# Ending2015a/dungeon_maps

Measured on NVIDIA B200. Metric: top-down maps/sec (batch 64, 640x480 depth + 16 semantic channels -> 400x400 maps), higher is better.
Workload: dtype f32

## Files before the change

dungeon_maps_b200/csrc/dm_labels.cu:

```cuda
#include <type_traits>

#include "dm_project.cuh"

namespace dm {

constexpr int kLblWarps = 8;
constexpr int kLblThreads = 32 * (kLblWarps + 1);
#ifndef DM_LBL_PROJ_J
#define DM_LBL_PROJ_J 1
#endif
constexpr int kLblProjJ = DM_LBL_PROJ_J;
constexpr int kLblTile = 128 * kLblWarps * kLblProjJ;
#ifndef DM_LBL_RES_K
#define DM_LBL_RES_K 2
#endif
constexpr int kLblResK = DM_LBL_RES_K;
constexpr int kLblResCells = 64 * kLblWarps * kLblResK;
#ifndef DM_LBL_RING
#define DM_LBL_RING 64
#endif
constexpr int kLblMaxRing = DM_LBL_RING;
constexpr int kLblList = 128 + 4;
constexpr uint32_t kKeyNegInf = 0x007fffffu;

struct LblPlan {
  int C, W2, CP, ring, lag, nsl;
  size_t slot_words, ctrl_bytes, flag_bytes;
  size_t workspace_bytes() const { return ctrl_bytes + flag_bytes + slot_words * 4 * (size_t)ring; }
};

static LblPlan make_lbl_plan(const DmProjCfg& cfg, int b) {
  LblPlan p{};
  p.C = cfg.C;
  p.W2 = (cfg.C + 1 <= 32) ? 1 : 2;
  p.CP = 1 + p.W2;
  const size_t M = (size_t)cfg.Mh * cfg.Mw;
  p.slot_words = (M * p.CP + 3) & ~(size_t)3;
  const int bb = b > 0 ? b : 1;
  p.ring = bb < kLblMaxRing ? bb : kLblMaxRing;
  if (p.ring < 2) p.ring = 2;
  p.lag = p.ring / 2;
  p.nsl = (int)((M + kSliceCells - 1) / kSliceCells);
  p.ctrl_bytes = ((size_t)(kCtrlWords + 2 * bb) * 4 + 255) & ~(size_t)255;
  p.flag_bytes = ((size_t)p.ring * p.nsl * kFlagStride * 4 + 255) & ~(size_t)255;
  return p;
}

struct LblDims {
  int C, CP, ring, lag, nsl, hasH;
  int vec_in;
  int vec_out;
  unsigned long long slot_words, ws_words;
};

struct LblItem {
  int kind, frame, idx, ok;
};

__device__ __forceinline__ uint32_t ld_stream_u32(const void* p) {
  uint32_t v;
  asm volatile("ld.global.nc.L1::no_allocate.u32 %0, [%1];" : "=r"(v) : "l"(p));
  return v;
}
__device__ __forceinline__ void red_or_u32(uint32_t* p, uint32_t v) {
  asm volatile("red.relaxed.gpu.global.or.b32 [%0], %1;" ::"l"(p), "r"(v) : "memory");
}

template <int W2>
using LblBits = std::conditional_t<W2 == 1, uint32_t, unsigned long long>;

struct LblQuad {
  float z[4];
  uint32_t lab, vm;
};

__device__ __forceinline__ LblQuad lbl_load_quad(const LblDims& d, const float* __restrict__ dframe,
                                                 const uint8_t* __restrict__ lframe, const uint8_t* __restrict__ vframe,
                                                 int n0, int N) {
  LblQuad q;
  q.z[0] = q.z[1] = q.z[2] = q.z[3] = 0.0f;
  q.lab = 0;
  q.vm = 0;
  if (n0 >= N) return q;
  if (d.vec_in && n0 + 3 < N) {
    const float4 z4 = ld_stream_f4(dframe + n0);
    q.z[0] = z4.x; q.z[1] = z4.y; q.z[2] = z4.z; q.z[3] = z4.w;
    q.lab = ld_stream_u32(lframe + n0);
    q.vm = vframe ? ld_stream_u32(vframe + n0) : 0x01010101u;
  } else {
#pragma unroll
    for (int k = 0; k < 4; ++k) {
      const bool in = n0 + k < N;
      q.z[k] = in ? ld_stream_f1(dframe + n0 + k) : 0.0f;
      q.lab |= (in ? (uint32_t)lframe[n0 + k] : 0u) << (8 * k);
      q.vm |= (in ? (vframe ? (uint32_t)(vframe[n0 + k] != 0) : 1u) : 0u) << (8 * k);
    }
  }
  return q;
}

template <int FAST, int W2>
__device__ __forceinline__ void lbl_proj_warp(const DmProjCfg& cfg, const LblDims& d, const DmProjSample& sp,
                                              const Rcps& rcp, const LblQuad& quad, int n0, int lane, uint32_t* list,
                                              uint32_t* __restrict__ acc, uint32_t slot_off,
                                              uint32_t* __restrict__ slot_flags) {
  using Bits = LblBits<W2>;
  const int N = cfg.H * cfg.W;
  int cl[4] = {-1, -1, -1, -1};
  float y[4] = {0.f, 0.f, 0.f, 0.f};
  Bits bt[4] = {0, 0, 0, 0};
  if (n0 < N) {
    const float* z = quad.z;
    const uint32_t lab = quad.lab, vm = quad.vm;
    const int r = n0 / cfg.W, c = n0 - r * cfg.W;
    if (FAST && c + 3 < cfg.W) {
      float xn[4];
#pragma unroll
      for (int k = 0; k < 4; ++k) xn[k] = div_by_rcp(__fsub_rn((float)(c + k), cfg.cx), cfg.fx, rcp.fx);
      const float yy = cfg.flip_h ? __fsub_rn((float)(cfg.H - 1), (float)r) : (float)r;
      const float yn = div_by_rcp(__fsub_rn(yy, cfg.cy), cfg.fy, rcp.fy);
      bool rowok = true;
      const int kb = cfg.clip_border;
      if (kb > 0) rowok = (r >= kb) && (r < cfg.H - kb);
#pragma unroll
      for (int k = 0; k < 4; ++k) {
        bool ok = rowok && (((vm >> (8 * k)) & 0xffu) != 0);
        if (kb > 0) ok = ok && (c + k >= kb) && (c + k < cfg.W - kb);
        cl[k] = pixel_cell_fast<FAST == 2, true>(cfg, sp, xn[k], yn, z[k], ok, &y[k], rcp.res);
      }
    } else {
      int rk = r, ck = c;
#pragma unroll
      for (int k = 0; k < 4; ++k) {
        cl[k] = pixel_cell(cfg, sp, rk, ck, z[k], ((vm >> (8 * k)) & 0xffu) != 0, &y[k]);
        if (++ck == cfg.W) { ck = 0; ++rk; }
      }
    }
#pragma unroll
    for (int k = 0; k < 4; ++k) {
      const int l = (int)((lab >> (8 * k)) & 0xffu);
      bt[k] = (Bits)1 << (l < cfg.C ? l : cfg.C);
    }
  }
  const bool p01 = (cl[0] >= 0) && (cl[0] == cl[1]);
  const bool p12 = (cl[1] >= 0) && (cl[1] == cl[2]);
  const bool p23 = (cl[2] >= 0) && (cl[2] == cl[3]);
  const bool t0 = (cl[0] >= 0) && !p01, t1 = (cl[1] >= 0) && !p12, t2 = (cl[2] >= 0) && !p23, t3 = cl[3] >= 0;
  y[1] = p01 ? fmaxf(y[0], y[1]) : y[1]; bt[1] = p01 ? (bt[0] | bt[1]) : bt[1];
  y[2] = p12 ? fmaxf(y[1], y[2]) : y[2]; bt[2] = p12 ? (bt[1] | bt[2]) : bt[2];
  y[3] = p23 ? fmaxf(y[2], y[3]) : y[3]; bt[3] = p23 ? (bt[2] | bt[3]) : bt[3];
// ... 460 lines not shown
```

dungeon_maps_b200/csrc/dm_project.cu:

```cuda
#include <cstdio>
#include <cstdlib>

#include <cuda.h>

#include "dm_project.cuh"

namespace dm {

constexpr int kProjThreads = 256;
constexpr int kResolveCells = 256;
#ifndef DM_MAX_RING
#define DM_MAX_RING 10
#endif
constexpr int kMaxRing = DM_MAX_RING;
constexpr size_t kRingBudgetBytes = (size_t)1 << 30;

struct ProjPlan {
  int Cv;
  int hasH;
  int CU;
  int CP;
  int rows;
  int tile;
  int ring;
  int lag;
  int nsl;
  size_t slot_words;
  size_t ctrl_bytes;
  size_t flag_bytes;
  size_t stage_bytes;
  size_t smem_tile;
  size_t smem_resolve;
  int ws_warps;
  int ws_groups;
  int ws_cg;
  int lean;
  int ws_r2d;
  size_t ws_stage_bytes;
  size_t smem_ws;
  size_t workspace_bytes() const { return ctrl_bytes + flag_bytes + slot_words * 4 * (size_t)ring; }
};

static int g_tile_rows = -1;
#ifndef DM_R2D_DEFAULT
#define DM_R2D_DEFAULT 0
#endif

static ProjPlan make_plan(const DmProjCfg& cfg, int b, int tile_rows = -1) {
  ProjPlan p{};
  p.Cv = cfg.C > 0 ? cfg.C : 1;
  p.hasH = (cfg.C > 0 && cfg.want_height) ? 1 : 0;
  p.CU = p.Cv + p.hasH;
  p.CP = (p.CU & 1) ? p.CU : p.CU + 1;
  p.rows = cfg.C + 1;
  const size_t M = (size_t)cfg.Mh * cfg.Mw;
  p.slot_words = (M * p.CP + 3) & ~(size_t)3;
  size_t ring = kRingBudgetBytes / (p.slot_words * 4);
  p.lean = cfg.C == 0 && g_tile_rows != -3;
  if (ring > (size_t)(p.lean ? 64 : kMaxRing)) ring = p.lean ? 64 : kMaxRing;
  if (ring > (size_t)(b > 0 ? b : 1)) ring = (size_t)(b > 0 ? b : 1);
  if (ring < 2) ring = 2;
  p.ring = (int)ring;
  p.lag = p.ring / 2;
  p.nsl = (int)((M + kSliceCells - 1) / kSliceCells);
  p.ctrl_bytes = ((size_t)(kCtrlWords + 2 * (b > 0 ? b : 1)) * 4 + 255) & ~(size_t)255;
  p.flag_bytes = ((size_t)p.ring * p.nsl * kFlagStride * 4 + 255) & ~(size_t)255;
  int tile = 1024;
  auto stage = [&](int t) { return (size_t)p.rows * (t + 4) * 4 + (size_t)t * 4; };
  while (tile > 128 && stage(tile) > (size_t)40 * 1024) tile >>= 1;
  p.tile = tile;
  p.stage_bytes = (stage(tile) + 127) & ~(size_t)127;
  p.smem_resolve = (size_t)kResolveCells * p.CP * 4;
  size_t st = p.stage_bytes > p.smem_resolve ? p.stage_bytes : ((p.smem_resolve + 127) & ~(size_t)127);
  p.stage_bytes = st;
  p.smem_tile = st + 256;
  auto ws_stage = [&](int ww, int rows) {
    size_t ws = ((size_t)rows * (128 * ww + 4) * 4 + (size_t)128 * ww * 4 + 127) & ~(size_t)127;
    const size_t ws_res = ((size_t)ww * 64 * p.CP * 4 + 127) & ~(size_t)127;
    return ws < ws_res ? ws_res : ws;
  };
  auto fits4 = [&](int ww, int rows) { return (ws_stage(ww, rows) + 256 + 1024) * 4 <= (size_t)228 * 1024; };
  p.ws_warps = 4;
  p.ws_groups = 1;
  if (!fits4(4, cfg.C + 1)) {
    p.ws_groups = (cfg.C + 23) / 24;
    p.ws_warps = 2;
  }
#ifdef DM_EXPERIMENT_KNOBS
  if (const char* e = getenv("DM_WS_WARPS")) {
    const int ww = atoi(e);
    if (ww == 2 || ww == 4) p.ws_warps = ww;
  }
  if (const char* e = getenv("DM_WS_GROUPS")) {
    const int g = atoi(e);
    if (g >= 1 && g <= 8) p.ws_groups = g;
  }
#endif
  if (cfg.C <= 0) p.ws_groups = 1;
  p.ws_cg = cfg.C > 0 ? (cfg.C + p.ws_groups - 1) / p.ws_groups : 0;
  p.ws_groups = cfg.C > 0 ? (cfg.C + p.ws_cg - 1) / p.ws_cg : 1;
  p.ws_r2d = tile_rows >= 0 ? tile_rows : g_tile_rows >= 0 ? g_tile_rows : DM_R2D_DEFAULT;
#ifdef DM_EXPERIMENT_KNOBS
  if (const char* e = getenv("DM_R2D")) if (tile_rows < 0) p.ws_r2d = atoi(e);
#endif
  if (p.ws_r2d != 0 && p.ws_r2d != 4 && p.ws_r2d != 8) p.ws_r2d = 0;
  if (p.ws_r2d == 8) {
    if (p.ws_groups == 1 && p.ws_warps == 4) p.ws_warps = 2; else p.ws_r2d = 4;
  }
  if (p.ws_r2d) {
    const size_t pw = (size_t)p.ws_r2d * 32 * p.ws_warps * 4;
    const size_t ws = (size_t)(p.ws_cg + 2) * pw;
    const size_t ws_res = ((size_t)p.ws_warps * 64 * p.CP * 4 + 127) & ~(size_t)127;
    p.ws_stage_bytes = ws < ws_res ? ws_res : ws;
    if (p.ws_cg > 256) p.ws_r2d = 0;
  }
  if (!p.ws_r2d) p.ws_stage_bytes = ws_stage(p.ws_warps, p.ws_cg + 1);
  p.smem_ws = p.ws_stage_bytes + 256;
  return p;
}

struct ProjDims {
  int Cv, hasH, CU, CP, rows, tile, ring, lag, nsl;
  unsigned long long slot_words;
  unsigned long long stage_bytes;
  int groups = 1, cg = 0;
  unsigned long long ws_words = 0;
};


__device__ __forceinline__ void phase_a(const uint8_t* __restrict__ vplane, const DmProjSample& sp,
                                        const DmProjCfg& cfg, int tile, int tile0, float* zrow, int* cells) {
  const int N = cfg.H * cfg.W;
  for (int q = threadIdx.x * 4; q < tile; q += kProjThreads * 4) {
    const int n0 = tile0 + q;
    int cl[4] = {-1, -1, -1, -1};
    float y[4] = {0.f, 0.f, 0.f, 0.f};
    if (n0 < N) {
      const float4 z4 = *reinterpret_cast<const float4*>(zrow + q);
      const float z[4] = {z4.x, z4.y, z4.z, z4.w};
      int r = n0 / cfg.W;
      int c = n0 - r * cfg.W;
#pragma unroll
      for (int k = 0; k < 4; ++k) {
        const bool ok = (n0 + k < N) && (vplane ? vplane[n0 + k] != 0 : true);
        cl[k] = pixel_cell(cfg, sp, r, c, z[k], ok, &y[k]);
        if (++c == cfg.W) { c = 0; ++r; }
      }
    }
    *reinterpret_cast<int4*>(cells + q) = make_int4(cl[0], cl[1], cl[2], cl[3]);
    *reinterpret_cast<float4*>(zrow + q) = make_float4(y[0], y[1], y[2], y[3]);
  }
}

template <bool IS_MIN>
__device__ __forceinline__ void emit_runs(const int* __restrict__ cells, const float* __restrict__ row,
                                          int beg, int end, float fill, uint32_t* __restrict__ acc_c, int CP) {
  int run_cell = -1;
  float run_v = fill;
  auto flush = [&]() {
    if (run_cell >= 0 && (IS_MIN ? (run_v < fill) : (run_v > fill)))
      atomicMax(acc_c + (size_t)run_cell * CP, IS_MIN ? ~enc(run_v) : enc(run_v));
  };
  auto visit = [&](int cl, float v) {
    if (cl >= 0) {
      if (cl != run_cell) {
        flush();
        run_cell = cl;
        run_v = fill;
      }
      run_v = IS_MIN ? fminf(run_v, v) : fmaxf(run_v, v);
    }
  };
  for (int i = beg; i < end; i += 4) {
    const int4 cl4 = *reinterpret_cast<const int4*>(cells + i);
    const float4 v4 = *reinterpret_cast<const float4*>(row + i);
    visit(cl4.x, v4.x);
    visit(cl4.y, v4.y);
    visit(cl4.z, v4.z);
    visit(cl4.w, v4.w);
  }
  flush();
}

// ... 139 lines not shown
  constexpr int RS = 128 * WW + 4;
  const int N = cfg.H * cfg.W;
  const int sb = cw * 128;
  const int q = sb + 4 * lane;
  const int n0 = it.tile0 + q;
  float* zrow = vals + nch * RS;
  int cl[4] = {-1, -1, -1, -1};
  float y[4] = {0.f, 0.f, 0.f, 0.f};
  if (n0 < N) {
    const float4 z4 = *reinterpret_cast<const float4*>(zrow + q);
    const float z[4] = {z4.x, z4.y, z4.z, z4.w};
    int c = it.c0 + q, r = it.r0;
    while (c >= cfg.W) { c -= cfg.W; ++r; }
    uint32_t vm = 0x01010101u;
    if (vplane) vm = *reinterpret_cast<const uint32_t*>(vplane + n0);
    if (FAST) {
      float xn[4];
#pragma unroll
      for (int k = 0; k < 4; ++k) xn[k] = div_by_rcp(__fsub_rn((float)(c + k), cfg.cx), cfg.fx, rcp.fx);
      const float yy = cfg.flip_h ? __fsub_rn((float)(cfg.H - 1), (float)r) : (float)r;
      const float yn = div_by_rcp(__fsub_rn(yy, cfg.cy), cfg.fy, rcp.fy);
      bool rowok = true;
      const int kb = cfg.clip_border;
      if (kb > 0) rowok = (r >= kb) && (r < cfg.H - kb);
#pragma unroll
      for (int k = 0; k < 4; ++k) {
        bool ok = rowok && (((vm >> (8 * k)) & 0xffu) != 0);
        if (kb > 0) ok = ok && (c + k >= kb) && (c + k < cfg.W - kb);
        cl[k] = pixel_cell_fast<FAST == 2, true>(cfg, sp, xn[k], yn, z[k], ok, &y[k], rcp.res);
      }
    } else {
#pragma unroll
      for (int k = 0; k < 4; ++k)
        cl[k] = pixel_cell(cfg, sp, r, c + k, z[k], ((vm >> (8 * k)) & 0xffu) != 0, &y[k]);
    }
  }
  const bool p01 = (cl[0] >= 0) && (cl[0] == cl[1]);
  const bool p12 = (cl[1] >= 0) && (cl[1] == cl[2]);
  const bool p23 = (cl[2] >= 0) && (cl[2] == cl[3]);
  const bool t0 = (cl[0] >= 0) && !p01, t1 = (cl[1] >= 0) && !p12, t2 = (cl[2] >= 0) && !p23, t3 = cl[3] >= 0;
  const int cnt = (int)t0 + (int)t1 + (int)t2 + (int)t3;
  int incl = cnt;
#pragma unroll
  for (int o = 1; o < 32; o <<= 1) {
    const int n = __shfl_up_sync(0xffffffffu, incl, o);
    if (lane >= o) incl += n;
  }
  const int total = __shfl_sync(0xffffffffu, incl, 31);
  const int padn = (4 - (total & 3)) & 3;
  const int o0 = sb + incl - cnt, o1 = o0 + (int)t0, o2 = o1 + (int)t1, o3 = o2 + (int)t2;
  if (t0) lcell[o0] = cl[0] * d.CP;
  if (t1) lcell[o1] = cl[1] * d.CP;
  if (t2) lcell[o2] = cl[2] * d.CP;
  if (t3) lcell[o3] = cl[3] * d.CP;
  {
    const int s0 = cl[0] >> 6, s1 = cl[1] >> 6, s2 = cl[2] >> 6, s3 = cl[3] >> 6;
    const int lastv = t3 ? s3 : t2 ? s2 : t1 ? s1 : t0 ? s0 : -1;
    int prev = __shfl_up_sync(0xffffffffu, lastv, 1);
    if (lane == 0) prev = -1;
    if (t0 && s0 != prev) st_flag(slot_flags + s0 * kFlagStride);
    prev = t0 ? s0 : prev;
    if (t1 && s1 != prev) st_flag(slot_flags + s1 * kFlagStride);
    prev = t1 ? s1 : prev;
    if (t2 && s2 != prev) st_flag(slot_flags + s2 * kFlagStride);
    prev = t2 ? s2 : prev;
    if (t3 && s3 != prev) st_flag(slot_flags + s3 * kFlagStride);
  }
  {
    const bool hmin = IS_MIN && cfg.C == 0;
    y[1] = p01 ? (hmin ? fminf(y[0], y[1]) : fmaxf(y[0], y[1])) : y[1];
    y[2] = p12 ? (hmin ? fminf(y[1], y[2]) : fmaxf(y[1], y[2])) : y[2];
    y[3] = p23 ? (hmin ? fminf(y[2], y[3]) : fmaxf(y[2], y[3])) : y[3];
    __syncwarp();
    if (t0) zrow[o0] = y[0];
    if (t1) zrow[o1] = y[1];
    if (t2) zrow[o2] = y[2];
    if (t3) zrow[o3] = y[3];
  }
  mbar_wait(full_vals, phase);
#ifdef DM_ABL_NOB
  return;
#endif
  [[maybe_unused]] const long long tp1 = DM_CLK();
#define DM_B1_ROW(ROW)                                                     \
  {                                                                        \
    float* row_ = (ROW);                                                   \
    float4 a = *reinterpret_cast<const float4*>(row_ + q);                 \
    a.y = p01 ? red2<IS_MIN>(a.x, a.y) : a.y;                              \
    a.z = p12 ? red2<IS_MIN>(a.y, a.z) : a.z;                              \
    a.w = p23 ? red2<IS_MIN>(a.z, a.w) : a.w;                              \
    __syncwarp();                                                          \
    if (t0) row_[o0] = a.x;                                                \
    if (t1) row_[o1] = a.y;                                                \
    if (t2) row_[o2] = a.z;                                                \
    if (t3) row_[o3] = a.w;                                                \
  }
  {
    int c = 0;
    for (; c + 4 <= nch; c += 4) {
      float* r0 = vals + c * RS;
      float4 a0 = *reinterpret_cast<const float4*>(r0 + q);
      float4 a1 = *reinterpret_cast<const float4*>(r0 + RS + q);
      float4 a2 = *reinterpret_cast<const float4*>(r0 + 2 * RS + q);
      float4 a3 = *reinterpret_cast<const float4*>(r0 + 3 * RS + q);
      a0.y = p01 ? red2<IS_MIN>(a0.x, a0.y) : a0.y; a1.y = p01 ? red2<IS_MIN>(a1.x, a1.y) : a1.y;
      a2.y = p01 ? red2<IS_MIN>(a2.x, a2.y) : a2.y; a3.y = p01 ? red2<IS_MIN>(a3.x, a3.y) : a3.y;
      a0.z = p12 ? red2<IS_MIN>(a0.y, a0.z) : a0.z; a1.z = p12 ? red2<IS_MIN>(a1.y, a1.z) : a1.z;
      a2.z = p12 ? red2<IS_MIN>(a2.y, a2.z) : a2.z; a3.z = p12 ? red2<IS_MIN>(a3.y, a3.z) : a3.z;
      a0.w = p23 ? red2<IS_MIN>(a0.z, a0.w) : a0.w; a1.w = p23 ? red2<IS_MIN>(a1.z, a1.w) : a1.w;
      a2.w = p23 ? red2<IS_MIN>(a2.z, a2.w) : a2.w; a3.w = p23 ? red2<IS_MIN>(a3.z, a3.w) : a3.w;
      __syncwarp();
      if (t0) { r0[o0] = a0.x; r0[RS + o0] = a1.x; r0[2 * RS + o0] = a2.x; r0[3 * RS + o0] = a3.x; }
      if (t1) { r0[o1] = a0.y; r0[RS + o1] = a1.y; r0[2 * RS + o1] = a2.y; r0[3 * RS + o1] = a3.y; }
      if (t2) { r0[o2] = a0.z; r0[RS + o2] = a1.z; r0[2 * RS + o2] = a2.z; r0[3 * RS + o2] = a3.z; }
      if (t3) { r0[o3] = a0.w; r0[RS + o3] = a1.w; r0[2 * RS + o3] = a2.w; r0[3 * RS + o3] = a3.w; }
    }
    for (; c < nch; ++c) DM_B1_ROW(vals + c * RS)
  }
#undef DM_B1_ROW
  __syncwarp();
  [[maybe_unused]] const long long tp2 = DM_CLK();
  const int total4 = total + padn;
  if (cfg.C > 0) {
    const int Cv = nch;
    const int cu_eff = Cv < 32 ? Cv : 32;
    const int streams = Cv <= 32 ? 32 / Cv : 1;
    const int passes = Cv <= 32 ? 1 : (Cv + 31) / 32;
    const int s = lane / cu_eff;
    const int per = ((total4 / 4 + streams - 1) / streams) * 4;
    const int beg = s * per;
    const int end = min(beg + per, total4);
    for (int pass = 0; pass < passes; ++pass) {
      const int c = pass * 32 + (lane - s * cu_eff);
      if (s >= streams || c >= Cv) continue;
      const float* row = vals + c * RS + sb;
      const int* lc = lcell + sb;
      const uint32_t off_c = slot_off + (uint32_t)(ch0 + c);
      const float fill = cfg.fill_value;
#ifdef DM_B2_BRANCHFREE
      if (beg >= end) continue;
      uint32_t pc = (uint32_t)lc[beg];
#else
      uint32_t pc = 0xffffffffu;
#endif
      float pv = fill;
      for (int i = beg; i < end; i += 4) {
        uint4 c4 = *reinterpret_cast<const uint4*>(lc + i);
        float4 v4 = *reinterpret_cast<const float4*>(row + i);
        if (i + 4 > total) {
          const int n = total - i;
          if (n < 2) { c4.y = c4.x; v4.y = fill; }
          if (n < 3) { c4.z = c4.y; v4.z = fill; }
          c4.w = c4.z; v4.w = fill;
        }
        const bool mp = pc == c4.x, m01 = c4.x == c4.y, m12 = c4.y == c4.z, m23 = c4.z == c4.w;
        red_key_if_run_ends<IS_MIN>(pc, c4.x, pv, fill, acc + (off_c + pc));
        v4.x = mp ? red2<IS_MIN>(pv, v4.x) : v4.x;
        v4.y = m01 ? red2<IS_MIN>(v4.x, v4.y) : v4.y;
        v4.z = m12 ? red2<IS_MIN>(v4.y, v4.z) : v4.z;
        v4.w = m23 ? red2<IS_MIN>(v4.z, v4.w) : v4.w;
        red_key_if_run_ends<IS_MIN>(c4.x, c4.y, v4.x, fill, acc + (off_c + c4.x));
        red_key_if_run_ends<IS_MIN>(c4.y, c4.z, v4.y, fill, acc + (off_c + c4.y));
        red_key_if_run_ends<IS_MIN>(c4.z, c4.w, v4.z, fill, acc + (off_c + c4.z));
        pc = c4.w;
        pv = v4.w;
      }
      red_key_if_run_ends<IS_MIN>(pc, 0xfffffffeu, pv, fill, acc + (off_c + pc));
    }
  }
  if ((d.hasH || cfg.C == 0) && ch0 == 0) {
    const bool hmin = IS_MIN && cfg.C == 0;
    const float hfill = cfg.C == 0 ? cfg.fill_value : -INFINITY;
    const uint32_t hoff = slot_off + (cfg.C == 0 ? 0u : (uint32_t)d.Cv);
    for (int base = 0; base < total; base += 32) {
      const int i = base + lane;
      const bool active = i < total;
      const uint32_t cellv = active ? (uint32_t)lcell[sb + i] : 0xffffffffu;
      float v = active ? zrow[sb + i] : hfill;
#pragma unroll
      for (int o = 1; o < 32; o <<= 1) {
        const float pv = __shfl_up_sync(0xffffffffu, v, o);
        const uint32_t pc = __shfl_up_sync(0xffffffffu, cellv, o);
        if (lane >= o && pc == cellv) v = hmin ? fminf(v, pv) : fmaxf(v, pv);
      }
      const uint32_t nc = __shfl_down_sync(0xffffffffu, cellv, 1);
      const bool last = lane == 31 || nc != cellv;
      const bool win = hmin ? (v < hfill) : (v > hfill);
      if (active && last && win) red_max_u32(acc + (hoff + cellv), hmin ? ~enc(v) : enc(v));
    }
  }
#ifdef DM_PROFILE
  [[maybe_unused]] const long long tp3 = DM_CLK();
  tprof[0] += tp1 - tp0; tprof[1] += tp2 - tp1; tprof[2] += tp3 - tp2; tprof[3] += total;
#endif
}

template <int FAST, bool IS_MIN, int WW, int R>
__device__ __forceinline__ void ws_proj_slice2d(const DmProjCfg& cfg, const ProjDims& d, const WsItem& it,
                                                const DmProjSample& sp, const Rcps& rcp,
                                                const uint8_t* __restrict__ vplane, float* vals, int* lcell,
                                                uint32_t* __restrict__ acc, uint32_t slot_off,
                                                uint32_t* __restrict__ slot_flags, int cw, int lane,
                                                uint64_t* full_vals, uint32_t phase, int ch0, int nch,
                                                long long* tprof) {
  [[maybe_unused]] const long long tp0 = DM_CLK();
  constexpr int TW = 32 * WW;
  constexpr int PW = R * TW;
  const int colt = (cw << 5) + lane;
  const int wbase = cw << 5;
  auto pos = [&](int i) { return (i >> 5) * TW + wbase + (i & 31); };
  float* zrow = vals + d.cg * PW;
  int cl[R];
  float y[R];
  {
    const int c = it.c0 + colt;
    const bool colok = c < cfg.W;
    float z[R];
#pragma unroll
    for (int k = 0; k < R; ++k) z[k] = zrow[k * TW + colt];
    const int kb = cfg.clip_border;
    bool ok[R];
#pragma unroll
    for (int k = 0; k < R; ++k) {
      const int r = it.r0 + k;
      ok[k] = colok && r < cfg.H;
      if (kb > 0) ok[k] = ok[k] && (r >= kb) && (r < cfg.H - kb) && (c >= kb) && (c < cfg.W - kb);
      if (vplane && ok[k]) ok[k] = vplane[(size_t)r * cfg.W + c] != 0;
    }
    if (FAST) {
      const float xn = div_by_rcp(__fsub_rn((float)c, cfg.cx), cfg.fx, rcp.fx);
#pragma unroll
      for (int k = 0; k < R; ++k) {
        const int r = it.r0 + k;
        const float yy = cfg.flip_h ? __fsub_rn((float)(cfg.H - 1), (float)r) : (float)r;
        const float yn = div_by_rcp(__fsub_rn(yy, cfg.cy), cfg.fy, rcp.fy);
        cl[k] = pixel_cell_fast<FAST == 2, true>(cfg, sp, xn, yn, z[k], ok[k], &y[k], rcp.res);
      }
    } else {
#pragma unroll
      for (int k = 0; k < R; ++k) {
        y[k] = 0.f;
        cl[k] = ok[k] ? pixel_cell(cfg, sp, it.r0 + k, c, z[k], true, &y[k]) : -1;
      }
    }
  }
  bool p[R], t[R];
#pragma unroll
  for (int k = 0; k < R; ++k) {
    p[k] = (k + 1 < R) && (cl[k] >= 0) && (cl[k] == cl[k + 1 < R ? k + 1 : k]);
    t[k] = (cl[k] >= 0) && !p[k];
  }
  int o[R];
  int total = 0;
  {
    const unsigned lt = (1u << lane) - 1u;
#pragma unroll
    for (int k = 0; k < R; ++k) {
      const unsigned bk = __ballot_sync(0xffffffffu, t[k]);
      o[k] = pos(total + __popc(bk & lt));
      total += __popc(bk);
    }
  }
  const int padn = (4 - (total & 3)) & 3;
#pragma unroll
  for (int k = 0; k < R; ++k)
    if (t[k]) lcell[o[k]] = cl[k] * d.CP;
  {
    int prev = -1;
#pragma unroll
    for (int k = 0; k < R; ++k) {
      const int sk = cl[k] >> 6;
      const int lk = __shfl_up_sync(0xffffffffu, t[k] ? sk : -1, 1);
      if (t[k] && sk != prev && (lane == 0 || sk != lk)) st_flag(slot_flags + sk * kFlagStride);
// ... 40 lines not shown
        for (int u = 0; u < CB; ++u)
          if (c + 4 * u < nch) {
#pragma unroll
            for (int k = 0; k < R; ++k)
              if (t[k]) pl[4 * u * PW + os[k]] = a[u][k];
          }
      }
    }
  }
  __syncwarp();
  [[maybe_unused]] const long long tp2 = DM_CLK();
  const int total4 = total + padn;
  if (cfg.C > 0) {
    const int Cv = nch;
    const int cu_eff = Cv < 32 ? Cv : 32;
    const int streams = Cv <= 32 ? 32 / Cv : 1;
    const int passes = Cv <= 32 ? 1 : (Cv + 31) / 32;
    const int s = lane / cu_eff;
    const int per = ((total4 / 4 + streams - 1) / streams) * 4;
    const int beg = s * per;
    const int end = min(beg + per, total4);
    for (int pass = 0; pass < passes; ++pass) {
      const int c = pass * 32 + (lane - s * cu_eff);
      if (s >= streams || c >= Cv) continue;
      const float* pl = vals + c * PW;
      const int swz = 4 * (c & 3);
      const uint32_t off_c = slot_off + (uint32_t)(ch0 + c);
      const float fill = cfg.fill_value;
      uint32_t pc = 0xffffffffu;
      float pv = fill;
      for (int i = beg; i < end; i += 4) {
        const int pi = pos(i);
        uint4 c4 = *reinterpret_cast<const uint4*>(lcell + pi);
        float4 v4 = *reinterpret_cast<const float4*>(pl + (pi ^ swz));
        if (i + 4 > total) {
          const int n = total - i;
          if (n < 2) { c4.y = c4.x; v4.y = fill; }
          if (n < 3) { c4.z = c4.y; v4.z = fill; }
          c4.w = c4.z; v4.w = fill;
        }
        const bool mp = pc == c4.x, m01 = c4.x == c4.y, m12 = c4.y == c4.z, m23 = c4.z == c4.w;
        red_key_if_run_ends<IS_MIN>(pc, c4.x, pv, fill, acc + (off_c + pc));
        v4.x = mp ? red2<IS_MIN>(pv, v4.x) : v4.x;
        v4.y = m01 ? red2<IS_MIN>(v4.x, v4.y) : v4.y;
        v4.z = m12 ? red2<IS_MIN>(v4.y, v4.z) : v4.z;
        v4.w = m23 ? red2<IS_MIN>(v4.z, v4.w) : v4.w;
        red_key_if_run_ends<IS_MIN>(c4.x, c4.y, v4.x, fill, acc + (off_c + c4.x));
        red_key_if_run_ends<IS_MIN>(c4.y, c4.z, v4.y, fill, acc + (off_c + c4.y));
        red_key_if_run_ends<IS_MIN>(c4.z, c4.w, v4.z, fill, acc + (off_c + c4.z));
        pc = c4.w;
        pv = v4.w;
      }
      red_key_if_run_ends<IS_MIN>(pc, 0xfffffffeu, pv, fill, acc + (off_c + pc));
    }
  }
  if ((d.hasH || cfg.C == 0) && ch0 == 0) {
    const bool hmin = IS_MIN && cfg.C == 0;
    const float hfill = cfg.C == 0 ? cfg.fill_value : -INFINITY;
    const uint32_t hoff = slot_off + (cfg.C == 0 ? 0u : (uint32_t)d.Cv);
    for (int base = 0; base < total; base += 32) {
      const int i = base + lane;
      const bool active = i < total;
      const int pi = pos(i);
      const uint32_t cellv = active ? (uint32_t)lcell[pi] : 0xffffffffu;
      float v = active ? zrow[pi] : hfill;
#pragma unroll
      for (int o2 = 1; o2 < 32; o2 <<= 1) {
        const float pv = __shfl_up_sync(0xffffffffu, v, o2);
        const uint32_t pc = __shfl_up_sync(0xffffffffu, cellv, o2);
        if (lane >= o2 && pc == cellv) v = hmin ? fminf(v, pv) : fmaxf(v, pv);
      }
      const uint32_t nc = __shfl_down_sync(0xffffffffu, cellv, 1);
      const bool last = lane == 31 || nc != cellv;
      const bool win = hmin ? (v < hfill) : (v > hfill);
      if (active && last && win) red_max_u32(acc + (hoff + cellv), hmin ? ~enc(v) : enc(v));
    }
  }
#ifdef DM_PROFILE
  [[maybe_unused]] const long long tp3 = DM_CLK();
  tprof[0] += tp1 - tp0; tprof[1] += tp2 - tp1; tprof[2] += tp3 - tp2; tprof[3] += total;
#endif
}

__device__ __forceinline__ bool ws_resolve_slice(uint32_t* __restrict__ acc_slot, const DmProjCfg& cfg,
                                                 const ProjDims& d, uint32_t* __restrict__ slot_flags, int frame,
                                                 int cell_tile, int tile_cells, int cw, int lane, uint32_t* wres,
                                                 float* __restrict__ topdown,
                                                 uint8_t* __restrict__ mask, float* __restrict__ height) {
  const int M = cfg.Mh * cfg.Mw;
  const int cell0 = cell_tile * tile_cells + cw * 64;
  const int ncell = min(64, M - cell0);
  if (ncell <= 0) return false;
  uint32_t* slice_flag = slot_flags + (size_t)(cell0 >> 6) * kFlagStride;
  const int nw = ncell * d.CP;
  const int nw4 = nw & ~3;
  uint32_t* src = acc_slot + (size_t)cell0 * d.CP;
  uint32_t any = 0;
  uint32_t flagged = 0;
  if (lane == 0) {
    flagged = __ldcg(slice_flag);
    if (flagged) __stcg(slice_flag, 0u);
  }
  flagged = __shfl_sync(0xffffffffu, flagged, 0);
  if (!flagged) {
    if (!(ncell == 64 && (M & 3) == 0))
      for (int k = lane; k < nw; k += 32) wres[k] = 0;
  } else {
  for (int base = 0; base < nw4; base += 512) {
    uint4 v[4];
#pragma unroll
    for (int u = 0; u < 4; ++u) {
      const int i = base + (u * 32 + lane) * 4;
      v[u] = i < nw4 ? __ldcg(reinterpret_cast<const uint4*>(src + i)) : make_uint4(0, 0, 0, 0);
    }
#pragma unroll
    for (int u = 0; u < 4; ++u) {
      const int i = base + (u * 32 + lane) * 4;
      const uint32_t nz = v[u].x | v[u].y | v[u].z | v[u].w;
      any |= nz;
      if (i < nw4) {
        if (nz) __stcg(reinterpret_cast<uint4*>(src + i), make_uint4(0, 0, 0, 0));
        *reinterpret_cast<uint4*>(wres + i) = v[u];
      }
    }
  }
  for (int k = nw4 + lane; k < nw; k += 32) {
    const uint32_t v = __ldcg(src + k);
    if (v) __stcg(src + k, 0u);
    wres[k] = v;
    any |= v;
  }
  }
  const bool occupied = __any_sync(0xffffffffu, any != 0);
  const size_t plane0 = (size_t)frame * d.Cv * M + cell0;
  if (!occupied && ncell == 64 && (M & 3) == 0) {
    const float f = cfg.fill_value;
    const float4 f4 = make_float4(f, f, f, f);
    for (int c = lane >> 4; c < d.Cv; c += 2) st_stream_f4(topdown + plane0 + (size_t)c * M + (lane & 15) * 4, f4);
    if ((M & 15) == 0) {
      for (int c = lane >> 2; c < d.Cv; c += 8) st_stream_u4(mask + plane0 + (size_t)c * M + (lane & 3) * 16, 0u);
    } else {
      for (int c = lane >> 4; c < d.Cv; c += 2) st_stream_u32(mask + plane0 + (size_t)c * M + (lane & 15) * 4, 0u);
    }
    if (d.hasH && lane < 16)
      st_stream_f4(height + (size_t)frame * M + cell0 + lane * 4, make_float4(-INFINITY, -INFINITY, -INFINITY, -INFINITY));
    return flagged != 0;
  }
  __syncwarp();
  for (int j = lane; j < ncell; j += 32) {
    const uint32_t* mine = wres + j * d.CP;
    float* tp = topdown + plane0 + j;
    uint8_t* mp = mask + plane0 + j;
    for (int c = 0; c < d.Cv; ++c) {
      const uint32_t k = mine[c];
      const float out = k ? dec_red(k, cfg.reduction) : cfg.fill_value;
      st_stream_f1(tp, out);
      st_stream_u8(mp, k ? 1 : 0);
      tp += M;
      mp += M;
    }
    if (d.hasH) {
      const uint32_t k = mine[d.Cv];
      st_stream_f1(height + (size_t)frame * M + cell0 + j, k ? dec(k) : -INFINITY);
    }
  }
  __syncwarp();
  return flagged != 0;
}

template <int FAST, bool IS_MIN, int WW, int R2D>
#ifndef DM_WS_MINB
#define DM_WS_MINB 0
#endif
__global__ void __launch_bounds__(32 * (WW + 1), (R2D == 4 && WW == 4) ? 6 : DM_WS_MINB)
proj_ws_kernel(const float* __restrict__ depth, const float* __restrict__ values,
               const uint8_t* __restrict__ valid, const DmProjSample* __restrict__ samples,
               const DmProjCfg cfg, const ProjDims d, int b, uint32_t* __restrict__ ctrl,
               uint32_t* __restrict__ flags, uint32_t* __restrict__ acc, float* __restrict__ topdown,
               uint8_t* __restrict__ mask, float* __restrict__ height, const ProjGuard guard,
               const __grid_constant__ CUtensorMap tmv, const __grid_constant__ CUtensorMap tmd) {
  extern __shared__ __align__(128) unsigned char smem[];
  constexpr int kWsWarps = WW, kWsTile = 128 * WW, kWsResolveCells = 64 * WW * kResK;
  constexpr int RS = kWsTile + 4;
  constexpr int TW = 32 * WW;
  constexpr int PW = (R2D ? R2D : 1) * TW;
  const Rcps rcp{__frcp_rn(cfg.map_res), __frcp_rn(cfg.fx), __frcp_rn(cfg.fy)};
  unsigned char* stage = smem;
  unsigned char* tail = smem + d.stage_bytes;
  uint64_t* full = reinterpret_cast<uint64_t*>(tail);
  uint64_t* empty = full + 1;
  uint64_t* full_vals = reinterpret_cast<uint64_t*>(tail + 24);
  WsItem* item = reinterpret_cast<WsItem*>(tail + 32);
  DmProjSample* sps = reinterpret_cast<DmProjSample*>(tail + 64);

  const int tid = threadIdx.x, lane = tid & 31, warp = tid >> 5;
  const int N = cfg.H * cfg.W, M = cfg.Mh * cfg.Mw;
  const int CBk = (cfg.W + TW - 1) / TW;
  const int P = (R2D ? ((cfg.H + R2D - 1) / (R2D ? R2D : 1)) * CBk : (N + kWsTile - 1) / kWsTile) * d.groups;
  const int R = (M + kWsResolveCells - 1) / kWsResolveCells;
  uint32_t* proj_done = ctrl + kCtrlWords;
  uint32_t* resolve_done = proj_done + b;
  uint32_t* occ_count = reinterpret_cast<uint32_t*>(tail + 16);

  int lag = d.lag;
  {
    const uint32_t hint = __ldcg(ctrl + 4);
    if (hint) {
      const float touched = (float)(hint - 1u) * (1.0f / 65536.0f) * (float)d.slot_words * 4.0f;
      const int fit = (int)fminf((float)(48u << 20) / fmaxf(touched, 1.0f), 64.0f) - 2;
      lag = max(min(2, d.lag), min(fit, d.lag));
    }
  }
  const int ahead = lag >= 3 ? 2 : 1;
  const int ring = min(d.ring, 2 * lag);
  const unsigned total = (unsigned)(b + lag) * (unsigned)(P + R);

  if (tid == 0) {
    *occ_count = 0;
    mbar_init(full, 1);
    mbar_init(full_vals, 1);
    mbar_init(empty, kWsWarps);
    asm volatile("fence.mbarrier_init.release.cluster;" ::: "memory");
  }
  __syncthreads();

  if (warp == kWsWarps) {
    const uint64_t policy = policy_evict_first();
    int pend_kind = kItemNone, pend_frame = 0;
    uint32_t fills = 0;
    [[maybe_unused]] long long pp[4] = {0, 0, 0, 0};
    unsigned raw0 = 0, raw1 = 0;
    if (lane == 0) {
      raw0 = atomicAdd(ctrl, 1u);
      if (ahead == 2) raw1 = atomicAdd(ctrl, 1u);
    }
    while (true) {
      [[maybe_unused]] const long long tq0 = DM_CLK();
      const unsigned t = __shfl_sync(0xffffffffu, raw0, 0);
      if (lane == 0) {
        if (ahead == 2) {
          raw0 = raw1;
          if (t < total) raw1 = atomicAdd(ctrl, 1u);
        } else if (t < total) {
          raw0 = atomicAdd(ctrl, 1u);
        }
      }
      WsItem it{};
      it.ok = 1;
      if (t >= total) {
        it.kind = kItemExit;
      } else {
        decode_ticket(t, b, P, R, lag, &it.kind, &it.frame, &it.idx);
      }
      const uint32_t* dep = nullptr;
      uint32_t dep_target = 0;
      uint32_t spw0 = 0, spw1 = 0;
      if (it.kind == kItemProj) {
// ... 476 lines not shown
```

dungeon_maps_b200/csrc/dm_project.cuh:

```cuda
#pragma once

#include "dm_common.cuh"

namespace dm {

constexpr int kSliceCells = 64;
#ifndef DM_FLAG_STRIDE
#define DM_FLAG_STRIDE 8
#endif
constexpr int kFlagStride = DM_FLAG_STRIDE;
constexpr int kCtrlWords = 512;
constexpr unsigned long long kSpinLimitNs = 4000000000ull;
#ifndef DM_SUSPEND_NS
#define DM_SUSPEND_NS 20000u
#endif

struct ProjGuard {
  unsigned long long spin_ns;
  uint32_t dep_bias;
  uint32_t* status;
};
ProjGuard proj_guard(int device);
bool take_timeout(int device);

// ... 47 lines not shown
__device__ __forceinline__ uint64_t policy_evict_first() {
  uint64_t p;
  asm volatile("createpolicy.fractional.L2::evict_first.b64 %0, 1.0;" : "=l"(p));
  return p;
}
__device__ __forceinline__ uint32_t ld_acquire(const uint32_t* p) {
  uint32_t v;
  asm volatile("ld.acquire.gpu.global.u32 %0, [%1];" : "=r"(v) : "l"(p) : "memory");
  return v;
}
__device__ __forceinline__ uint32_t ld_relaxed(const uint32_t* p) {
  uint32_t v;
  asm volatile("ld.relaxed.gpu.global.u32 %0, [%1];" : "=r"(v) : "l"(p) : "memory");
  return v;
}
__device__ __forceinline__ unsigned long long globaltimer() {
  unsigned long long t;
  asm volatile("mov.u64 %0, %globaltimer;" : "=l"(t));
  return t;
}
__device__ __forceinline__ bool wait_count(const uint32_t* counter, uint32_t target, uint32_t* ctrl,
                                           unsigned long long spin_ns) {
  if (ld_acquire(counter) >= target) return true;
  const unsigned long long t0 = globaltimer();
  while (ld_acquire(counter) < target) {
    __nanosleep(64);
    if (globaltimer() - t0 > spin_ns) {
      atomicExch(ctrl + 2, 1u);
      return false;
    }
  }
  return true;
}

__device__ __forceinline__ void red_release_add1(uint32_t* p) {
  asm volatile("red.release.gpu.global.add.u32 [%0], 1;" ::"l"(p) : "memory");
}

__device__ __forceinline__ void scrub_after_timeout(uint32_t* ctrl, uint32_t* flags, unsigned long long words, int tid,
                                                    int nthreads, uint32_t* status) {
  if (__ldcg(ctrl + 2) == 0u) return;
  uint4* w4 = reinterpret_cast<uint4*>(flags);
  for (unsigned long long i = tid; i < words / 4; i += nthreads) __stcg(w4 + i, make_uint4(0u, 0u, 0u, 0u));
  __threadfence();
  if (tid == 0 && status) {
    asm volatile("st.relaxed.sys.global.u32 [%0], %1;" ::"l"(status), "r"(1u) : "memory");
    __threadfence_system();
  }
}

enum { kItemProj = 0, kItemResolve = 1, kItemNone = 2, kItemExit = 3 };

__device__ __forceinline__ void decode_ticket(unsigned t, int b, int P, int R, int lag, int* kind, int* frame,
                                              int* idx) {
  const unsigned per = (unsigned)(P + R);
  const int s = (int)(t / per);
  const int j = (int)(t - (unsigned)s * per);
  const unsigned rb0 = (unsigned)(((unsigned long long)j * (unsigned)R) / per);
  const unsigned rb1 = (unsigned)(((unsigned long long)(j + 1) * (unsigned)R) / per);
  if (rb1 > rb0) {
    *kind = kItemResolve;
    *idx = (int)rb0;
  } else {
    *kind = kItemProj;
    *idx = j - (int)rb0;
  }
  *frame = *kind == kItemProj ? s : s - lag;
  if (*frame < 0 || *frame >= b) *kind = kItemNone;
}

__device__ __forceinline__ void mbar_arrive(uint64_t* bar) {
  asm volatile("mbarrier.arrive.shared::cta.b64 _, [%0];" ::"r"(smem_u32(bar)) : "memory");
}

__device__ __forceinline__ void st_flag(uint32_t* p) {
  asm volatile("st.relaxed.gpu.global.u32 [%0], %1;" ::"l"(p), "r"(1u) : "memory");
}
__device__ __forceinline__ void red_max_u32(uint32_t* p, uint32_t v) {
#ifdef DM_ABL_NORED
  asm volatile("" ::"l"(p), "r"(v) : "memory");
#else
  asm volatile("red.relaxed.gpu.global.max.u32 [%0], %1;" ::"l"(p), "r"(v) : "memory");
#endif
}
template <bool IS_MIN>
__device__ __forceinline__ void red_key_if_run_ends(uint32_t ca, uint32_t cb, float v, float fill, uint32_t* p) {
  const uint32_t key = IS_MIN ? ~enc(v) : enc(v);
#ifdef DM_ABL_NORED
  asm volatile("" ::"r"(ca), "r"(cb), "f"(v), "f"(fill), "l"(p), "r"(key) : "memory");
#elif defined(DM_B2_BRANCHFREE)
  {
    const bool on = (ca != cb) && (IS_MIN ? (v < fill) : (v > fill));
    asm volatile("red.relaxed.gpu.global.max.u32 [%0], %1;" ::"l"(p), "r"(on ? key : 0u) : "memory");
  }
#elif defined(DM_ABL_REDVAR)
  {
    const int ln = threadIdx.x & 31;
    bool on = (ca != cb) && (IS_MIN ? (v < fill) : (v > fill));
#if DM_ABL_REDVAR == 2
    on = on && ((ln & 1) == 0);
#elif DM_ABL_REDVAR == 4
    on = on && ((ln & 15) == 0);
#endif
#if DM_ABL_REDVAR == 3
    p = reinterpret_cast<uint32_t*>((reinterpret_cast<unsigned long long>(p) & ~0xfffffffull) | (reinterpret_cast<unsigned long long>(p) & 0xffffcull));
#endif
#if DM_ABL_REDVAR == 1
    if (on) asm volatile("st.relaxed.gpu.global.u32 [%0], %1;" ::"l"(p), "r"(key) : "memory");
#else
    if (on) asm volatile("red.relaxed.gpu.global.max.u32 [%0], %1;" ::"l"(p), "r"(key) : "memory");
#endif
  }
#else
  if (IS_MIN)
    asm volatile(
        "{\n\t.reg .pred p;\n\t"
        "setp.ne.u32 p, %0, %1;\n\t"
        "setp.lt.and.f32 p, %2, %3, p;\n\t"
        "@p red.relaxed.gpu.global.max.u32 [%4], %5;\n\t}" ::"r"(ca), "r"(cb), "f"(v), "f"(fill), "l"(p), "r"(key) : "memory");
  else
    asm volatile(
        "{\n\t.reg .pred p;\n\t"
        "setp.ne.u32 p, %0, %1;\n\t"
        "setp.gt.and.f32 p, %2, %3, p;\n\t"
        "@p red.relaxed.gpu.global.max.u32 [%4], %5;\n\t}" ::"r"(ca), "r"(cb), "f"(v), "f"(fill), "l"(p), "r"(key) : "memory");
#endif
}
__device__ __forceinline__ void red_max_u32_if(bool pred, uint32_t* p, uint32_t v) {
  asm volatile(
      "{\n\t.reg .pred p;\n\t"
      "setp.ne.b32 p, %0, 0;\n\t"
      "@p red.global.max.u32 [%1], %2;\n\t}" ::"r"((int)pred), "l"(p), "r"(v) : "memory");
}

__device__ __forceinline__ float div_by_rcp(float x, float res, float rres) {
  const float q0 = __fmul_rn(x, rres);
  const float q1 = __fmaf_rn(__fmaf_rn(-q0, res, x), rres, q0);
  return __fmaf_rn(__fmaf_rn(-q1, res, x), rres, q1);
}

template <bool GLOBAL, bool RCP_DIV = false>
__device__ __forceinline__ int pixel_cell_fast(const DmProjCfg& cfg, const DmProjSample& sp, float xn, float yn,
                                               float z, bool ok, float* y_out, float rres = 0.0f) {
  if (cfg.has_trunc_depth_max) ok = ok && (z <= cfg.trunc_depth_max);
  if (cfg.has_trunc_depth_min) ok = ok && (z >= cfg.trunc_depth_min);
  const float X = __fmul_rn(xn, z), Y = __fmul_rn(yn, z);
  const float* Rl = sp.to_local.R;
  float ly = __fmaf_rn(Rl[7], z, __fmul_rn(Rl[4], Y));
  float lz = __fmaf_rn(Rl[8], z, __fmul_rn(Rl[5], Y));
  ly = __fadd_rn(ly, sp.to_local.t[1]);
  if (cfg.has_trunc_height_max) ok = ok && (ly <= cfg.trunc_height_max);
  float gx = X, gz = lz;
  if (GLOBAL) {
    const float* Rg = sp.to_global.R;
    gx = __fadd_rn(__fmaf_rn(Rg[6], lz, __fmul_rn(Rg[0], X)), sp.to_global.t[0]);
    gz = __fadd_rn(__fmaf_rn(Rg[8], lz, __fmul_rn(Rg[2], X)), sp.to_global.t[2]);
  }
  float xf, zf;
  if (RCP_DIV) {
    const float res = cfg.map_res;
    const float xb = __fadd_rn(div_by_rcp(gx, res, rres), sp.width_offset);
    float zb = __fadd_rn(div_by_rcp(gz, res, rres), sp.height_offset);
    if (cfg.flip_h) zb = __fsub_rn((float)(cfg.Mh - 1), zb);
    xf = floorf(__fadd_rn(xb, 0.5f));
    zf = floorf(__fadd_rn(zb, 0.5f));
  } else {
// ... 20 lines not shown
```

Measured before the change: 137,100.

## Add binary-value presence bitmask path for semantic channel projection

Checks at runtime whether every semantic value in a warp's tile is exactly 0 or 1. When so, it packs per-pixel channel bits into one presence word per cell group and issues a single red.or per cell run instead of per-channel red.max operations. The resolve stage then expands the presence bits back into per-channel keys. This widens the cell slot by the number of groups, rescales the ring cap to keep memory similar, changes lag rounding, and sets a min-blocks launch bound for the R2D=0 path. The aim is to cut global atomic traffic for one-hot or binary labels, at the cost of extra detection work and a larger slot.

After: 139,200 (median of 6 runs). 1.02x the previous value.

```diff
diff --git a/dungeon_maps_b200/csrc/dm_labels.cu b/dungeon_maps_b200/csrc/dm_labels.cu
--- a/dungeon_maps_b200/csrc/dm_labels.cu
+++ b/dungeon_maps_b200/csrc/dm_labels.cu
@@ -62,10 +62,6 @@
   asm volatile("ld.global.nc.L1::no_allocate.u32 %0, [%1];" : "=r"(v) : "l"(p));
   return v;
 }
-__device__ __forceinline__ void red_or_u32(uint32_t* p, uint32_t v) {
-  asm volatile("red.relaxed.gpu.global.or.b32 [%0], %1;" ::"l"(p), "r"(v) : "memory");
-}
-
 template <int W2>
 using LblBits = std::conditional_t<W2 == 1, uint32_t, unsigned long long>;
 
diff --git a/dungeon_maps_b200/csrc/dm_project.cu b/dungeon_maps_b200/csrc/dm_project.cu
--- a/dungeon_maps_b200/csrc/dm_project.cu
+++ b/dungeon_maps_b200/csrc/dm_project.cu
@@ -1,5 +1,6 @@
 #include <cstdio>
 #include <cstdlib>
+#include <type_traits>
 
 #include <cuda.h>
 
@@ -51,17 +52,48 @@
   p.Cv = cfg.C > 0 ? cfg.C : 1;
   p.hasH = (cfg.C > 0 && cfg.want_height) ? 1 : 0;
   p.CU = p.Cv + p.hasH;
-  p.CP = (p.CU & 1) ? p.CU : p.CU + 1;
   p.rows = cfg.C + 1;
   const size_t M = (size_t)cfg.Mh * cfg.Mw;
+  auto ws_rows = [&](int ww, int rows) {
+    return ((size_t)rows * (128 * ww + 4) * 4 + (size_t)128 * ww * 4 + 127) & ~(size_t)127;
+  };
+  auto ws_stage = [&](int ww, int rows) {
+    const size_t ws = ws_rows(ww, rows);
+    const size_t ws_res = ((size_t)ww * 64 * p.CP * 4 + 127) & ~(size_t)127;
+    return ws < ws_res ? ws_res : ws;
+  };
+  auto fits4 = [&](int ww, int rows) { return (ws_rows(ww, rows) + 256 + 1024) * 4 <= (size_t)228 * 1024; };
+  p.ws_warps = 4;
+  p.ws_groups = 1;
+  if (!fits4(4, cfg.C + 1)) {
+    p.ws_groups = (cfg.C + 23) / 24;
+    p.ws_warps = 2;
+  }
+#ifdef DM_EXPERIMENT_KNOBS
+  if (const char* e = getenv("DM_WS_WARPS")) {
+    const int ww = atoi(e);
+    if (ww == 2 || ww == 4) p.ws_warps = ww;
+  }
+  if (const char* e = getenv("DM_WS_GROUPS")) {
+    const int g = atoi(e);
+    if (g >= 1 && g <= 8) p.ws_groups = g;
+  }
+#endif
+  if (cfg.C <= 0) p.ws_groups = 1;
+  p.ws_cg = cfg.C > 0 ? (cfg.C + p.ws_groups - 1) / p.ws_groups : 0;
+  p.ws_groups = cfg.C > 0 ? (cfg.C + p.ws_cg - 1) / p.ws_cg : 1;
+  const int cp_keys = (p.CU & 1) ? p.CU : p.CU + 1;
+  const int cell_words = p.CU + (cfg.C > 0 ? p.ws_groups : 0);
+  p.CP = (cell_words & 1) ? cell_words : cell_words + 1;
   p.slot_words = (M * p.CP + 3) & ~(size_t)3;
   size_t ring = kRingBudgetBytes / (p.slot_words * 4);
   p.lean = cfg.C == 0 && g_tile_rows != -3;
-  if (ring > (size_t)(p.lean ? 64 : kMaxRing)) ring = p.lean ? 64 : kMaxRing;
+  const size_t cap = p.lean ? 64 : ((size_t)kMaxRing * cp_keys + p.CP / 2) / p.CP;
+  if (ring > cap) ring = cap;
   if (ring > (size_t)(b > 0 ? b : 1)) ring = (size_t)(b > 0 ? b : 1);
   if (ring < 2) ring = 2;
   p.ring = (int)ring;
-  p.lag = p.ring / 2;
+  p.lag = (p.ring + 1) / 2;
   p.nsl = (int)((M + kSliceCells - 1) / kSliceCells);
   p.ctrl_bytes = ((size_t)(kCtrlWords + 2 * (b > 0 ? b : 1)) * 4 + 255) & ~(size_t)255;
   p.flag_bytes = ((size_t)p.ring * p.nsl * kFlagStride * 4 + 255) & ~(size_t)255;
@@ -74,31 +106,6 @@
   size_t st = p.stage_bytes > p.smem_resolve ? p.stage_bytes : ((p.smem_resolve + 127) & ~(size_t)127);
   p.stage_bytes = st;
   p.smem_tile = st + 256;
-  auto ws_stage = [&](int ww, int rows) {
-    size_t ws = ((size_t)rows * (128 * ww + 4) * 4 + (size_t)128 * ww * 4 + 127) & ~(size_t)127;
-    const size_t ws_res = ((size_t)ww * 64 * p.CP * 4 + 127) & ~(size_t)127;
-    return ws < ws_res ? ws_res : ws;
-  };
-  auto fits4 = [&](int ww, int rows) { return (ws_stage(ww, rows) + 256 + 1024) * 4 <= (size_t)228 * 1024; };
-  p.ws_warps = 4;
-  p.ws_groups = 1;
-  if (!fits4(4, cfg.C + 1)) {
-    p.ws_groups = (cfg.C + 23) / 24;
-    p.ws_warps = 2;
-  }
-#ifdef DM_EXPERIMENT_KNOBS
-  if (const char* e = getenv("DM_WS_WARPS")) {
-    const int ww = atoi(e);
-    if (ww == 2 || ww == 4) p.ws_warps = ww;
-  }
-  if (const char* e = getenv("DM_WS_GROUPS")) {
-    const int g = atoi(e);
-    if (g >= 1 && g <= 8) p.ws_groups = g;
-  }
-#endif
-  if (cfg.C <= 0) p.ws_groups = 1;
-  p.ws_cg = cfg.C > 0 ? (cfg.C + p.ws_groups - 1) / p.ws_groups : 0;
-  p.ws_groups = cfg.C > 0 ? (cfg.C + p.ws_cg - 1) / p.ws_cg : 1;
   p.ws_r2d = tile_rows >= 0 ? tile_rows : g_tile_rows >= 0 ? g_tile_rows : DM_R2D_DEFAULT;
 #ifdef DM_EXPERIMENT_KNOBS
   if (const char* e = getenv("DM_R2D")) if (tile_rows < 0) p.ws_r2d = atoi(e);
@@ -404,6 +411,7 @@
   return;
 #endif
   [[maybe_unused]] const long long tp1 = DM_CLK();
+  uint32_t nbo = 0, nbt = 0;
 #define DM_B1_ROW(ROW)                                                     \
   {                                                                        \
     float* row_ = (ROW);                                                   \
@@ -411,6 +419,7 @@
     a.y = p01 ? red2<IS_MIN>(a.x, a.y) : a.y;                              \
     a.z = p12 ? red2<IS_MIN>(a.y, a.z) : a.z;                              \
     a.w = p23 ? red2<IS_MIN>(a.z, a.w) : a.w;                              \
+    not01(a, nbo, nbt);                                                    \
     __syncwarp();                                                          \
     if (t0) row_[o0] = a.x;                                                \
     if (t1) row_[o1] = a.y;                                                \
@@ -431,6 +440,7 @@
       a2.z = p12 ? red2<IS_MIN>(a2.y, a2.z) : a2.z; a3.z = p12 ? red2<IS_MIN>(a3.y, a3.z) : a3.z;
       a0.w = p23 ? red2<IS_MIN>(a0.z, a0.w) : a0.w; a1.w = p23 ? red2<IS_MIN>(a1.z, a1.w) : a1.w;
       a2.w = p23 ? red2<IS_MIN>(a2.z, a2.w) : a2.w; a3.w = p23 ? red2<IS_MIN>(a3.z, a3.w) : a3.w;
+      not01(a0, nbo, nbt); not01(a1, nbo, nbt); not01(a2, nbo, nbt); not01(a3, nbo, nbt);
       __syncwarp();
       if (t0) { r0[o0] = a0.x; r0[RS + o0] = a1.x; r0[2 * RS + o0] = a2.x; r0[3 * RS + o0] = a3.x; }
       if (t1) { r0[o1] = a0.y; r0[RS + o1] = a1.y; r0[2 * RS + o1] = a2.y; r0[3 * RS + o1] = a3.y; }
@@ -442,8 +452,9 @@
 #undef DM_B1_ROW
   __syncwarp();
   [[maybe_unused]] const long long tp2 = DM_CLK();
+  const bool bin = cfg.C > 0 && nch <= 31 && __all_sync(0xffffffffu, ((nbo & ~0x3f800000u) | nbt) == 0u);
   const int total4 = total + padn;
-  if (cfg.C > 0) {
+  if (cfg.C > 0 && !bin) {
     const int Cv = nch;
     const int cu_eff = Cv < 32 ? Cv : 32;
     const int streams = Cv <= 32 ? 32 / Cv : 1;
@@ -490,27 +501,46 @@
       red_key_if_run_ends<IS_MIN>(pc, 0xfffffffeu, pv, fill, acc + (off_c + pc));
     }
   }
-  if ((d.hasH || cfg.C == 0) && ch0 == 0) {
-    const bool hmin = IS_MIN && cfg.C == 0;
-    const float hfill = cfg.C == 0 ? cfg.fill_value : -INFINITY;
-    const uint32_t hoff = slot_off + (cfg.C == 0 ? 0u : (uint32_t)d.Cv);
+  const bool hrow = (d.hasH || cfg.C == 0) && ch0 == 0;
+  auto runlet_pass = [&](auto pres) {
+    constexpr bool PRES = decltype(pres)::value;
+    const bool c0 = !PRES && cfg.C == 0;
+    const bool hmin = IS_MIN && c0;
+    const float hfill = c0 ? cfg.fill_value : -INFINITY;
+    const uint32_t hoff = slot_off + (c0 ? 0u : (uint32_t)d.Cv);
+    const uint32_t poff = slot_off + (uint32_t)(d.CU + (PRES ? ch0 / d.cg : 0));
     for (int base = 0; base < total; base += 32) {
       const int i = base + lane;
       const bool active = i < total;
       const uint32_t cellv = active ? (uint32_t)lcell[sb + i] : 0xffffffffu;
       float v = active ? zrow[sb + i] : hfill;
+      uint32_t pw = 0;
+      if (PRES && active) {
+        for (int c = nch - 1; c >= 0; --c) pw = (pw << 1) | (__float_as_uint(vals[c * RS + sb + i]) >> 29);
+        if (IS_MIN) pw = ~pw & ((1u << nch) - 1u);
+      }
 #pragma unroll
       for (int o = 1; o < 32; o <<= 1) {
         const float pv = __shfl_up_sync(0xffffffffu, v, o);
         const uint32_t pc = __shfl_up_sync(0xffffffffu, cellv, o);
-        if (lane >= o && pc == cellv) v = hmin ? fminf(v, pv) : fmaxf(v, pv);
+        uint32_t pp = 0;
+        if (PRES) pp = __shfl_up_sync(0xffffffffu, pw, o);
+        if (lane >= o && pc == cellv) {
+          v = hmin ? fminf(v, pv) : fmaxf(v, pv);
+          if (PRES) pw |= pp;
+        }
       }
       const uint32_t nc = __shfl_down_sync(0xffffffffu, cellv, 1);
       const bool last = lane == 31 || nc != cellv;
       const bool win = hmin ? (v < hfill) : (v > hfill);
-      if (active && last && win) red_max_u32(acc + (hoff + cellv), hmin ? ~enc(v) : enc(v));
-    }
-  }
+      if (hrow && active && last && win) red_max_u32(acc + (hoff + cellv), hmin ? ~enc(v) : enc(v));
+      if (PRES && active && last) red_or_u32(acc + (poff + cellv), pw | 0x80000000u);
+    }
+  };
+  if (bin)
+    runlet_pass(std::true_type{});
+  else if (hrow)
+    runlet_pass(std::false_type{});
 #ifdef DM_PROFILE
   [[maybe_unused]] const long long tp3 = DM_CLK();
   tprof[0] += tp1 - tp0; tprof[1] += tp2 - tp1; tprof[2] += tp3 - tp2; tprof[3] += total;
@@ -717,6 +747,23 @@
 #endif
 }
 
+__device__ __noinline__ void fold_presence(uint32_t* wres, int ncell, int lane, int CP, int CU, int Cv, int cg,
+                                           float fill, int mn) {
+  const float vb = mn ? 0.0f : 1.0f, vw = mn ? 1.0f : 0.0f;
+  const uint32_t KB = better(vb, fill, mn) ? enc_red(vb, mn) : 0u;
+  const uint32_t KW = better(vw, fill, mn) ? enc_red(vw, mn) : 0u;
+  for (int j = lane; j < ncell; j += 32) {
+    uint32_t* mine = wres + j * CP;
+    for (int c0 = 0, g = 0; c0 < Cv; c0 += cg, ++g) {
+      uint32_t pw = mine[CU + g];
+      if (pw >> 31) {
+        const int c1 = min(c0 + cg, Cv);
+        for (int c = c0; c < c1; ++c, pw >>= 1) mine[c] = max(mine[c], (pw & 1u) ? KB : KW);
+      }
+    }
+  }
+}
+
 __device__ __forceinline__ bool ws_resolve_slice(uint32_t* __restrict__ acc_slot, const DmProjCfg& cfg,
                                                  const ProjDims& d, uint32_t* __restrict__ slot_flags, int frame,
                                                  int cell_tile, int tile_cells, int cw, int lane, uint32_t* wres,
@@ -782,6 +829,7 @@
     return flagged != 0;
   }
   __syncwarp();
+  if (cfg.C > 0) fold_presence(wres, ncell, lane, d.CP, d.CU, d.Cv, d.cg, cfg.fill_value, cfg.reduction);
   for (int j = lane; j < ncell; j += 32) {
     const uint32_t* mine = wres + j * d.CP;
     float* tp = topdown + plane0 + j;
@@ -807,7 +855,7 @@
 #ifndef DM_WS_MINB
 #define DM_WS_MINB 0
 #endif
-__global__ void __launch_bounds__(32 * (WW + 1), (R2D == 4 && WW == 4) ? 6 : DM_WS_MINB)
+__global__ void __launch_bounds__(32 * (WW + 1), (R2D == 4 && WW == 4) ? 6 : R2D == 0 ? 65536 / (64 * 32 * (WW + 1)) : DM_WS_MINB)
 proj_ws_kernel(const float* __restrict__ depth, const float* __restrict__ values,
                const uint8_t* __restrict__ valid, const DmProjSample* __restrict__ samples,
                const DmProjCfg cfg, const ProjDims d, int b, uint32_t* __restrict__ ctrl,
diff --git a/dungeon_maps_b200/csrc/dm_project.cuh b/dungeon_maps_b200/csrc/dm_project.cuh
--- a/dungeon_maps_b200/csrc/dm_project.cuh
+++ b/dungeon_maps_b200/csrc/dm_project.cuh
@@ -153,6 +153,18 @@
 #else
   asm volatile("red.relaxed.gpu.global.max.u32 [%0], %1;" ::"l"(p), "r"(v) : "memory");
 #endif
+}
+__device__ __forceinline__ void red_or_u32(uint32_t* p, uint32_t v) {
+#ifdef DM_ABL_NORED
+  asm volatile("" ::"l"(p), "r"(v) : "memory");
+#else
+  asm volatile("red.relaxed.gpu.global.or.b32 [%0], %1;" ::"l"(p), "r"(v) : "memory");
+#endif
+}
+__device__ __forceinline__ void not01(const float4& a, uint32_t& o, uint32_t& t) {
+  o |= __float_as_uint(a.x) | __float_as_uint(a.y) | __float_as_uint(a.z) | __float_as_uint(a.w);
+  t |= __float_as_uint(__fmaf_rn(-a.x, a.x, a.x)) | __float_as_uint(__fmaf_rn(-a.y, a.y, a.y)) |
+       __float_as_uint(__fmaf_rn(-a.z, a.z, a.z)) | __float_as_uint(__fmaf_rn(-a.w, a.w, a.w));
 }
 template <bool IS_MIN>
 __device__ __forceinline__ void red_key_if_run_ends(uint32_t ca, uint32_t cb, float v, float fill, uint32_t* p) {
```
